# radian628/raymarching-engine

Measured on AMD Instinct MI355X. Metric: Mpixels/sec at 3840x2160 Mandelbulb, higher is better.
Workload: dtype f32

## Files before the change

include/hip_raymarch.h:

```cpp
#ifndef HIP_RAYMARCH_H
#define HIP_RAYMARCH_H

#include <stddef.h>
#include <stdint.h>

#ifndef RM_API
#define RM_API __attribute__((visibility("default")))
#endif

#ifdef __cplusplus
extern "C" {
#endif

#define RM_ABI_VERSION 8

#define RM_MAX_BOUNCES 10
#define RM_MAX_LIGHTS 10
#define RM_MAX_PRIMS 256

enum {
  RM_OK = 0,
  RM_ERR_INVALID = 1,
  RM_ERR_DEVICE = 2,
  RM_ERR_NO_DEVICE = 3
// ... 85 lines not shown
typedef struct RmSceneDesc {
  int32_t kind;
  int32_t nprims;
  const RmPrim* prims;
  float params[16];
  RmMaterial material;
  int32_t nsurfaces;
  int32_t reserved;
  const RmSurface* surfaces;
} RmSceneDesc;

RM_API void rm_material_default(RmMaterial* m);


typedef struct rm_ctx rm_ctx;
typedef struct rm_scene rm_scene;
typedef struct rm_fb rm_fb;

typedef struct RmRect {
  int32_t x, y, w, h;
} RmRect;

enum {
  RM_RENDER_STRICT = 0,
  RM_RENDER_FAST = 1,
  RM_RENDER_COLOR_ONLY = 2,
  RM_RENDER_MEGAKERNEL = 4,
  RM_RENDER_WAVEFRONT = 16,
  RM_RENDER_NO_COST_CLASSES = 8,
  RM_RENDER_NO_OVERLAP = 32,
  RM_RENDER_NO_FAR_JUMP = 64,
  RM_RENDER_NO_CULL = 128
};

enum { RM_PLANE_COLOR = 0, RM_PLANE_NORMAL_DOF = 1, RM_PLANE_ALBEDO_DEPTH = 2 };


RM_API int rm_ctx_create(int device, rm_ctx** out);
RM_API void rm_ctx_destroy(rm_ctx* ctx);
RM_API const char* rm_last_error(const rm_ctx* ctx);
RM_API int rm_ctx_set_stream(rm_ctx* ctx, void* hip_stream);
RM_API int rm_ctx_set_samples_in_flight(rm_ctx* ctx, int n);
RM_API const char* rm_ctx_last_warning(const rm_ctx* ctx);
RM_API int rm_ctx_set_sample_batch(rm_ctx* ctx, int n);
RM_API int rm_ctx_set_cost_order(rm_ctx* ctx, int on);
RM_API int rm_ctx_set_retire_eps(rm_ctx* ctx, float eps);
RM_API int rm_ctx_set_gl_stack(rm_ctx* ctx, int on);
RM_API int rm_ctx_set_cull_min_pixels(rm_ctx* ctx, long long pixels);
RM_API int rm_ctx_set_cull_budget(rm_ctx* ctx, size_t bytes);
RM_API int rm_ctx_cull_stats(const rm_ctx* ctx, unsigned long long* out4);
RM_API int rm_debug_counters(rm_ctx* ctx, unsigned long long* out16, int reset);

RM_API int rm_debug_cull_cell(const RmSceneDesc* desc, const double* centre, double radius, double margin, unsigned long long* out_words);
enum { RM_PIPELINE_NONE = 0, RM_PIPELINE_PIXEL_KERNEL = 1, RM_PIPELINE_WAVEFRONT = 2 };
RM_API int rm_ctx_last_pipeline(const rm_ctx* ctx);
RM_API int rm_device_memory(rm_ctx* ctx, size_t* free_bytes, size_t* total_bytes);
RM_API int rm_sync(rm_ctx* ctx);
RM_API int rm_abi_version(void);


RM_API int rm_scene_create(rm_ctx* ctx, const RmSceneDesc* desc, rm_scene** out);
RM_API void rm_scene_destroy(rm_scene* scene);


RM_API int rm_fb_create(rm_ctx* ctx, int width, int height, int row_begin, int row_count, rm_fb** out);
RM_API int rm_fb_create_striped(rm_ctx* ctx, int width, int height, int stripe_rows, int parts, int part,
                         void* color, void* normal_dof, void* albedo_depth, rm_fb** out);
RM_API int rm_fb_rows(const rm_fb* fb);
RM_API int rm_fb_width(const rm_fb* fb);
RM_API int rm_fb_height(const rm_fb* fb);
RM_API int rm_fb_wrap(rm_ctx* ctx, int width, int height, int row_begin, int row_count,
               void* color, void* normal_dof, void* albedo_depth, rm_fb** out);
RM_API int rm_fb_clear(rm_fb* fb);
RM_API void rm_fb_destroy(rm_fb* fb);
RM_API int rm_fb_download(rm_fb* fb, int plane, float* host);
RM_API int rm_fb_upload(rm_fb* fb, int plane, const float* host);
RM_API void* rm_fb_device_ptr(rm_fb* fb, int plane);

RM_API int rm_buffer_create(rm_ctx* ctx, size_t bytes, void** device_ptr);
RM_API int rm_buffer_destroy(rm_ctx* ctx, void* device_ptr);
RM_API int rm_buffer_download(rm_ctx* ctx, const void* device_ptr, void* host, size_t bytes);
RM_API int rm_buffer_upload(rm_ctx* ctx, void* device_ptr, const void* host, size_t bytes);


RM_API int rm_render_sample(rm_ctx* ctx, rm_scene* scene, rm_fb* fb, const RmUniforms* uniforms,
                     const RmRect* tile, int flags);

RM_API int rm_render_samples(rm_ctx* ctx, rm_scene* scene, rm_fb* fb, const RmUniforms* uniforms,
                      const float* rand_noise_pairs, int count, const RmRect* tile, int flags);

RM_API int rm_render_timed(rm_ctx* ctx, rm_scene* scene, rm_fb* fb, const RmUniforms* uniforms,
                    int count, const RmRect* tile, int flags, float* ms_per_launch);


enum { RM_PROBE_SDF = 0, RM_PROBE_CAST_RAY = 1, RM_PROBE_NORMAL = 2, RM_PROBE_MATERIAL = 3, RM_PROBE_CAST_STEPS = 4, RM_PROBE_CAST_SHADOW = 5 };
RM_API int rm_probe(rm_ctx* ctx, rm_scene* scene, int what, const float* in, int n, float param,
             int flags, float* out);

RM_API int rm_probe_camera(rm_ctx* ctx, const RmUniforms* uniforms, int width, int height, float* out);

RM_API int rm_probe_rng(rm_ctx* ctx, const RmUniforms* uniforms, int width, int height, int count, float* out);

enum { RM_MATH_SIN = 0, RM_MATH_COS = 1, RM_MATH_LOG = 2, RM_MATH_EXP = 3, RM_MATH_POW = 4, RM_MATH_ACOS = 5, RM_MATH_ATAN2 = 6, RM_MATH_TAN = 7,
       RM_MATH_POW_PAIR_NM1 = 8, RM_MATH_POW_PAIR_N = 9, RM_MATH_SINCOS_S = 10, RM_MATH_SINCOS_C = 11, RM_MATH_SQRT = 12, RM_MATH_DIV = 13, RM_MATH_COUNT = 14 };
RM_API int rm_probe_math(rm_ctx* ctx, int fn, const float* a, const float* b, int n, float* out);

// ... 25 lines not shown
```

raymarching-engine_amd/csrc/rm_api.hip:

```cpp
#include <hip/hip_runtime.h>

#include <cmath>
#include <cstdio>
#include <cstdlib>
#include <cstring>
#include <limits>
#include <mutex>
#include <new>
#include <string>
#include <unordered_map>
#include <vector>

#include "../../include/hip_raymarch.h"
#include "rm_params.hpp"

#ifndef RM_WITH_WAVEFRONT
#define RM_WITH_WAVEFRONT 0
#endif

#define RM_SP_MAX 8

extern "C" {
hipError_t rm_gl_launch_pixels(const void* kparams, hipStream_t stream);
hipError_t rm_gl_launch_probe(const void* probe_params, hipStream_t stream);
// ... 415 lines not shown
    reach = std::fmax(reach, std::fmax(std::fabs(lo[a]), std::fabs(hi[a])));
    build->centre[a] = 0.5 * (lo[a] + hi[a]);
  }
  half = 1.1 * half + kmax + 1e-3;
  if (!(half < 1e6) || !(reach < 1e6)) return false;
  int levels = 1;
  while (levels < RM_CULL_MAX_LEVELS && 1.2e-7 * (n + 8) * 1.74 * std::ldexp(half, levels) < 2.0 * half) levels++;
  if (smooth_spheres && levels > RM_CULL_SMOOTH_LEVELS) levels = RM_CULL_SMOOTH_LEVELS;
  build->half0 = half;
  build->reach = reach;
  build->nprims = n;
  const int cells = smooth_spheres ? (n >= 32 ? RM_CULL_N_SMOOTH : RM_CULL_N_SMOOTH / 2) : RM_CULL_N;
  build->n = cells;
  build->n_outer = smooth_spheres ? cells / RM_CULL_OUTER_DIV : cells;
  build->levels = levels;
  build->words = (n + 63) / 64;
  for (int a = 0; a < 3; a++) g->centre[a] = (float)build->centre[a];
  g->inv_half0 = (float)(1.0 / half);
  g->scale0 = (float)(cells / (2.0 * half));
  g->n = cells;
  g->n_outer = build->n_outer;
  g->levels = levels;
  g->words = build->words;
  return true;
}

int rm_debug_cull_cell(const RmSceneDesc* desc, const double* centre, double radius, double margin, unsigned long long* out_words) {
  if (!desc || !centre || !out_words || desc->kind != RM_SCENE_TABLE || desc->nprims < 1 || desc->nprims > RM_MAX_PRIMS || !desc->prims) return RM_ERR_INVALID;
  for (int i = 0; i < desc->nprims; i++) {
    const int type = desc->prims[i].type & 0xff;
    if ((type != RM_PRIM_SPHERE && type != RM_PRIM_BOX) || ((desc->prims[i].type >> 8) & 0xff) > RM_OP_INTERSECT) return RM_ERR_INVALID;
  }
  rm_cull_cell(desc->prims, desc->nprims, (desc->nprims + 63) / 64, centre, radius, margin, out_words);
  return RM_OK;
}

static void kifs_far_field(const RmSceneDesc* desc, DevScene* dev) {
  dev->far_end = 0;
  dev->far_r2 = 0.0f;
  const double iters = desc->params[RM_P_KIFS_ITERATIONS], s = desc->params[RM_P_KIFS_SCALE], off = std::fabs((double)desc->params[RM_P_KIFS_OFFSET]);
  if (!(s > 0.05 && s <= 0.9) || !(iters >= 0.0 && iters <= 64.0) || !(off < 1e6)) return;
  if (desc->kind == RM_SCENE_KIFS_BOX) {
    if (std::pow(s, std::ceil(iters)) < 1e-15) return;
    const double r = 2.0 * std::sqrt(3.0) * (off * s / (1.0 - s) + 1.0) + 1.0;
    dev->far_r2 = (float)(r * r);
    dev->far_end = 1;
  } else {
    const double r = 9999.0 + 1.01 * (off * s / (1.0 - s) + 1.0) + 2.0;
    dev->far_r2 = (float)(r * r);
    dev->far_end = 3;
  }
}

int rm_scene_create(rm_ctx* ctx, const RmSceneDesc* desc, rm_scene** out) {
  if (!ctx || !desc || !out) return fail(ctx, RM_ERR_INVALID, "rm_scene_create: NULL argument");
  *out = nullptr;
  char buf[256];
  if (desc->kind < 0 || desc->kind >= RM_SCENE_KIND_COUNT) {
    std::snprintf(buf, sizeof buf, "scene: unknown kind %d", desc->kind);
    return fail(ctx, RM_ERR_INVALID, buf);
  }
  if (!finite_all(desc->params, 16)) return fail(ctx, RM_ERR_INVALID, "scene: non-finite parameter");
  if (desc->material.sky_axis < 0 || desc->material.sky_axis > 2) return fail(ctx, RM_ERR_INVALID, "scene: material.sky_axis must be 0, 1 or 2");
  if (desc->nsurfaces < 0 || desc->nsurfaces > RM_MAX_SURFACES || (desc->nsurfaces > 0 && (!desc->surfaces || desc->kind != RM_SCENE_TABLE))) {
    std::snprintf(buf, sizeof buf, "scene: 0..%d surfaces, for a primitive table (got %d)", RM_MAX_SURFACES, desc->nsurfaces);
    return fail(ctx, RM_ERR_INVALID, buf);
  }
  for (int i = 0; i < desc->nsurfaces; i++)
    if (!finite_all(reinterpret_cast<const float*>(&desc->surfaces[i]), 12)) return fail(ctx, RM_ERR_INVALID, "scene: non-finite surface value");
  if (desc->kind == RM_SCENE_TABLE) {
    if (desc->nprims < 1 || desc->nprims > RM_MAX_PRIMS || !desc->prims) {
      std::snprintf(buf, sizeof buf, "scene: primitive table needs 1..%d rows (got %d)", RM_MAX_PRIMS, desc->nprims);
      return fail(ctx, RM_ERR_INVALID, buf);
    }
    int shapes = 0, kind_of_rows = -1;
    for (int i = 0; i < desc->nprims; i++) {
      const RmPrim& p = desc->prims[i];
      const int type = p.type & 0xff, op = (p.type >> 8) & 0xff;
      if (type > RM_PRIM_PLANE || op > RM_OP_SMOOTH_INTERSECT || (p.type >> 24) != 0) {
        std::snprintf(buf, sizeof buf, "scene: row %d: unknown primitive/operator 0x%x", i, p.type);
        return fail(ctx, RM_ERR_INVALID, buf);
      }
      const int surface = (p.type >> 16) & 0xff;
      if (type == RM_PRIM_KIND) {
        const int kind = (int)p.size[0];
        if ((float)kind != p.size[0] || (kind != RM_SCENE_MANDELBULB && kind != RM_SCENE_SPHERE_LATTICE)) {
          std::snprintf(buf, sizeof buf, "scene: row %d: a kind row evaluates RM_SCENE_MANDELBULB or RM_SCENE_SPHERE_LATTICE (size[0] = %g)", i, (double)p.size[0]);
          return fail(ctx, RM_ERR_INVALID, buf);
        }
        if (kind_of_rows >= 0 && kind_of_rows != kind) return fail(ctx, RM_ERR_INVALID, "scene: the kind rows of a table evaluate ONE kind (its parameters are the scene's parameter block)");
        kind_of_rows = kind;
        if (kind == RM_SCENE_MANDELBULB && !(desc->params[RM_P_BULB_ITERATIONS] >= 0.0f && desc->params[RM_P_BULB_ITERATIONS] <= 64.0f))
          return fail(ctx, RM_ERR_INVALID, "scene: mandelbulb iterations must be in 0..64");
        if (kind == RM_SCENE_SPHERE_LATTICE && !(desc->params[RM_P_LATTICE_PERIOD] > 0.0f)) return fail(ctx, RM_ERR_INVALID, "scene: the lattice's period must be > 0");
      }
      const bool shape = type != RM_PRIM_REPEAT && type != RM_PRIM_FOLD;
      if (surface > desc->nsurfaces || (surface != 0 && !shape)) {
        std::snprintf(buf, sizeof buf, "scene: row %d: surface %d of %d (only shape rows name a surface)", i, surface, desc->nsurfaces);
        return fail(ctx, RM_ERR_INVALID, buf);
      }
      if (!finite_all(p.center, 3) || !finite_all(p.size, 3) || !std::isfinite(p.k)) {
        std::snprintf(buf, sizeof buf, "scene: row %d: non-finite value", i);
        return fail(ctx, RM_ERR_INVALID, buf);
      }
      if (type == RM_PRIM_REPEAT && !(p.size[0] > 0.0f && p.size[1] > 0.0f && p.size[2] > 0.0f)) {
        std::snprintf(buf, sizeof buf, "scene: row %d: repeat needs a period > 0 on every axis", i);
// ... 2 lines not shown
      if (type == RM_PRIM_FOLD && !(p.k > 0.0f)) {
        std::snprintf(buf, sizeof buf, "scene: row %d: fold needs scale > 0", i);
        return fail(ctx, RM_ERR_INVALID, buf);
      }
      if (shape && (op == RM_OP_SMOOTH_UNION || op == RM_OP_SMOOTH_SUBTRACT || op == RM_OP_SMOOTH_INTERSECT) && !(p.k > 0.0f) && shapes > 0) {
        std::snprintf(buf, sizeof buf, "scene: row %d: smooth %s needs k > 0", i, op == RM_OP_SMOOTH_UNION ? "union" : op == RM_OP_SMOOTH_SUBTRACT ? "subtraction" : "intersection");
        return fail(ctx, RM_ERR_INVALID, buf);
      }
      if ((type == RM_PRIM_TORUS || type == RM_PRIM_CYLINDER) && !(p.size[0] >= 0.0f && p.size[1] >= 0.0f)) {
        std::snprintf(buf, sizeof buf, "scene: row %d: a torus / cylinder needs radii (and a half height) >= 0", i);
        return fail(ctx, RM_ERR_INVALID, buf);
      }
      if (type == RM_PRIM_PLANE && !(p.size[0] != 0.0f || p.size[1] != 0.0f || p.size[2] != 0.0f)) {
        std::snprintf(buf, sizeof buf, "scene: row %d: a plane needs a normal", i);
        return fail(ctx, RM_ERR_INVALID, buf);
      }
      shapes += shape ? 1 : 0;
    }
    if (shapes == 0) return fail(ctx, RM_ERR_INVALID, "scene: the table has no shape row (sphere / box), only domain operators");
  } else if (desc->kind == RM_SCENE_MANDELBULB) {
    if (!(desc->params[RM_P_BULB_ITERATIONS] >= 0.0f && desc->params[RM_P_BULB_ITERATIONS] <= 64.0f))
      return fail(ctx, RM_ERR_INVALID, "scene: mandelbulb iterations must be in 0..64");
  } else if (desc->kind == RM_SCENE_SPHERE_GRID || desc->kind == RM_SCENE_MENGER || desc->kind == RM_SCENE_KIFS_TREE ||
             desc->kind == RM_SCENE_KIFS_BOX) {
    const int slot = desc->kind == RM_SCENE_SPHERE_GRID ? RM_P_GRID_ITERATIONS : desc->kind == RM_SCENE_MENGER ? RM_P_MENGER_ITERATIONS : RM_P_KIFS_ITERATIONS;
    if (!(desc->params[slot] <= 64.0f)) return fail(ctx, RM_ERR_INVALID, "scene: fractal iterations must be <= 64");
  }
  rm_scene* s = new (std::nothrow) rm_scene();
  if (!s) return fail(ctx, RM_ERR_DEVICE, "out of host memory");
  s->ctx = ctx;
  s->dev.kind = desc->kind;
  s->dev.nprims = desc->kind == RM_SCENE_TABLE ? desc->nprims : 0;
  if (desc->kind == RM_SCENE_TABLE) {
    bool spheres_smooth = true, domain = false, boxes = false, surfaces = false, kinds = false, more = false;
    for (int i = 0; i < desc->nprims; i++) {
      const int type = desc->prims[i].type & 0xff, op = (desc->prims[i].type >> 8) & 0xff;
      if (((desc->prims[i].type >> 16) & 0xff) != 0) surfaces = true;
      if (type != RM_PRIM_SPHERE || (i > 0 && op != RM_OP_SMOOTH_UNION)) spheres_smooth = false;
      if (type == RM_PRIM_REPEAT || type == RM_PRIM_FOLD) domain = true;
      if (type == RM_PRIM_BOX || type == RM_PRIM_TORUS || type == RM_PRIM_CYLINDER || type == RM_PRIM_PLANE) boxes = true;
      if (type == RM_PRIM_KIND) kinds = true;
      if (type > RM_PRIM_KIND || op > RM_OP_INTERSECT) more = true;
    }
    s->dev.table_flags = (spheres_smooth ? RM_TABLE_SPHERES_SMOOTH : 0) | (domain ? RM_TABLE_HAS_DOMAIN : 0) | (boxes || kinds ? 0 : RM_TABLE_NO_BOXES) |
                         (surfaces ? RM_TABLE_HAS_SURFACES : 0) | (kinds ? RM_TABLE_HAS_KIND : 0) | (more ? RM_TABLE_MORE : 0);
    if (spheres_smooth && desc->nprims >= 2 && desc->nprims * 3 <= RM_MAX_PRIMS * 2) {
      bool one_k = true;
      for (int i = 2; i < desc->nprims; i++) one_k = one_k && desc->prims[i].k == desc->prims[1].k;
      if (one_k) s->dev.table_flags |= RM_TABLE_UNIFORM_K;
    }
  }
  if (desc->kind == RM_SCENE_TABLE) table_far_field(desc, &s->dev);
  if (desc->kind == RM_SCENE_KIFS_BOX || desc->kind == RM_SCENE_KIFS_TREE) kifs_far_field(desc, &s->dev);
  if (desc->kind == RM_SCENE_SPHERE_GRID) {
    const float* c = &desc->params[RM_P_GRID_CENTER];
    const double r = 2.0 * (std::sqrt((double)c[0] * c[0] + (double)c[1] * c[1] + (double)c[2] * c[2]) + std::fabs((double)desc->params[RM_P_GRID_BIG_SIZE])) + 1.0;
    if (r < 1e9) { s->dev.far_r2 = (float)(r * r); s->dev.far_end = 1; }
  }
  std::memcpy(s->dev.p, desc->params, sizeof s->dev.p);
  if (s->dev.table_flags & RM_TABLE_UNIFORM_K) {
    s->dev.p[0] = desc->prims[1].k;
    s->dev.p[1] = 0.5f * (1.0f / desc->prims[1].k);
  }
  s->dev.mat = desc->material;
  (void)hipSetDevice(ctx->device);
  if (s->dev.nprims > 0) {
    const size_t bytes = sizeof(RmPrim) * (size_t)s->dev.nprims;
    hipError_t e = hipMalloc(reinterpret_cast<void**>(&s->d_prims), bytes);
    if (e == hipSuccess) e = hipMemcpy(s->d_prims, desc->prims, bytes, hipMemcpyHostToDevice);
    if (e != hipSuccess) {
      if (s->d_prims) (void)hipFree(s->d_prims);
      delete s;
      return fail(ctx, RM_ERR_DEVICE, std::string("rm_scene_create: ") + hipGetErrorString(e));
    }
    s->dev.prims = s->d_prims;
  }
  if (desc->kind == RM_SCENE_TABLE) {
    CullGrid g;
    CullBuild build;
    if (table_cull_params(desc, &g, &build)) {
      s->cull_wanted = true;
      s->cull_grid = g;
      s->cull_build = build;
    }
  }
  if (s->dev.table_flags & RM_TABLE_HAS_SURFACES) {
    RmSurface all[RM_MAX_SURFACES + 1];
    const RmMaterial& m = desc->material;
    all[0] = RmSurface{{m.diffuse[0], m.diffuse[1], m.diffuse[2]}, m.roughness, {m.specular[0], m.specular[1], m.specular[2]}, m.subsurface,
                       {m.subsurface_color[0], m.subsurface_color[1], m.subsurface_color[2]}, m.ior};
    for (int i = 0; i < desc->nsurfaces; i++) all[i + 1] = desc->surfaces[i];
    const size_t bytes = sizeof(RmSurface) * (size_t)(desc->nsurfaces + 1);
    hipError_t e = hipMalloc(reinterpret_cast<void**>(&s->d_surfaces), bytes);
    if (e == hipSuccess) e = hipMemcpy(s->d_surfaces, all, bytes, hipMemcpyHostToDevice);
    if (e != hipSuccess) {
      if (s->d_surfaces) (void)hipFree(s->d_surfaces);
      if (s->d_prims) (void)hipFree(s->d_prims);
      delete s;
      return fail(ctx, RM_ERR_DEVICE, std::string("rm_scene_create: ") + hipGetErrorString(e));
    }
    s->dev.surfaces = s->d_surfaces;
    s->dev.nsurfaces = desc->nsurfaces;
  }
  *out = s;
  return RM_OK;
}
// ... 1088 lines not shown
```

raymarching-engine_amd/csrc/rm_device.hpp:

```cpp
#pragma once

#include <hip/hip_runtime.h>

#include "../../include/hip_raymarch.h"
#include "rm_params.hpp"

namespace rm {
#ifdef RM_LANE_STATS
static __device__ unsigned long long g_lane_stats[4];
#endif


#define RM_DEV __device__ __forceinline__

struct v3 {
  float x, y, z;
};

RM_DEV v3 V(float x, float y, float z) { return v3{x, y, z}; }
RM_DEV v3 operator+(v3 a, v3 b) { return V(a.x + b.x, a.y + b.y, a.z + b.z); }
RM_DEV v3 operator-(v3 a, v3 b) { return V(a.x - b.x, a.y - b.y, a.z - b.z); }
RM_DEV v3 operator*(v3 a, v3 b) { return V(a.x * b.x, a.y * b.y, a.z * b.z); }
RM_DEV v3 operator*(v3 a, float s) { return V(a.x * s, a.y * s, a.z * s); }
RM_DEV v3 adds(v3 a, float s) { return V(a.x + s, a.y + s, a.z + s); }
// ... 883 lines not shown
        else pow8_round_next(z, dr, pos, rho2, r2);
#ifdef RM_LANE_STATS
        rounds++;
#endif
      }
    } else {
      for (int i = 1; i < iterations; i++) {
        if (r2 > bail2) break;
        if (i == iterations - 1) dr = pow8_round_dr(dr, r2);
        else pow8_round_next(z, dr, pos, rho2, r2);
      }
    }
#ifdef RM_LANE_STATS
    lane_stats(rounds);
#endif
    return pow8_distance(r2, dr);
  }
#ifdef RM_LANE_STATS
  static RM_DEV void lane_stats(int rounds) {
    const unsigned long long act = ballot(true);
    unsigned long long lane_rounds = 0, wave_rounds = 0;
    for (int r = 1; r <= 8; r++) {
      const unsigned long long m = ballot(rounds >= r);
      lane_rounds += __popcll(m);
      wave_rounds += m != 0ull ? 1 : 0;
    }
    if ((int)__lane_id() == __ffsll((long long)act) - 1) {
      atomicAdd(&g_lane_stats[0], lane_rounds);
      atomicAdd(&g_lane_stats[1], wave_rounds * 64ull);
      atomicAdd(&g_lane_stats[2], (unsigned long long)__popcll(act));
      atomicAdd(&g_lane_stats[3], 64ull);
    }
  }
#endif
  static RM_DEV float eval_pow8(const DevScene& sc, v3 pos) {
    return (int)sc.p[RM_P_BULB_ITERATIONS] == 8 ? eval_pow8_n<8>(sc, pos) : eval_pow8_n<0>(sc, pos);
  }
  template <class M>
  static RM_DEV float eval(const DevScene& sc, const SceneLds&, v3 p) {
    if (M::fast && sc.p[RM_P_BULB_POWER] == 8.0f) return eval_pow8(sc, p);
    return eval_generic<M>(sc, p);
  }
  static constexpr int far_jump_steps = 30;
  static RM_DEV bool far_jump_applies(const DevScene& sc) { return sc.p[RM_P_BULB_ITERATIONS] >= 1.0f && sc.p[RM_P_BULB_BAILOUT] >= 0.0f; }
  static RM_DEV bool far_jump(const DevScene& sc, v3 p, v3 dir, int left, v3& end) {
    const float bail2 = sc.p[RM_P_BULB_BAILOUT] * sc.p[RM_P_BULB_BAILOUT];
    const float r2 = FM::fma(p.z, p.z, pow8_rho2(p));
    return far_jump_at(p, dir, left, r2, RM_BUILD_FAST && sc.p[RM_P_BULB_POWER] == 8.0f ? bail2 : 1.001f * bail2, end);
  }
  static RM_DEV bool far_jump_at(v3 p, v3 dir, int left, float r2, float bail2, v3& end) {
    if (!(r2 > gmax(bail2, 4.0f) && r2 < 1e30f) || left < (r2 >= 1e12f ? 16 : (r2 >= 1e4f ? 22 : far_jump_steps))) return false;
    const float s = dot<FM>(p, dir), dd = dot<FM>(dir, dir);
    if (!(s >= 0.0f && dd > 0.98f && dd < 1.02f)) return false;
    v3 e = dir * __builtin_inff();
    if (e.x != e.x || e.y != e.y || e.z != e.z) e = V(e.x + e.y + e.z, e.x + e.y + e.z, e.x + e.y + e.z);
    end = e;
    return true;
  }
  template <int ITERS>
  static RM_DEV bool pow8_eval_or_jump(const DevScene& sc, v3 p, v3 dir, int left, bool jump, float& d, v3& end) {
    const float bail2 = sc.p[RM_P_BULB_BAILOUT] * sc.p[RM_P_BULB_BAILOUT];
    const float rho2 = pow8_rho2(p);
    const float r2 = FM::fma(p.z, p.z, rho2);
    if (ITERS != 8 && (int)sc.p[RM_P_BULB_ITERATIONS] < 1) { d = pow8_distance(0.0f, 1.0f); return false; }
    if (r2 > bail2) {
      if (jump && far_jump_at(p, dir, left, r2, bail2, end)) return true;
#ifdef RM_LANE_STATS
      lane_stats(0);
#endif
      d = pow8_distance_far(r2);
      return false;
    }
    d = pow8_near<ITERS>(sc, p, rho2, r2, bail2);
    return false;
  }

  static constexpr bool has_cost_classes = true;
  static RM_DEV bool nonfinite_normal_is_nan(const DevScene&) { return true; }
  static constexpr int cheap_cap = 2;
  template <class M>
  static RM_DEV bool eval_cheap(const DevScene& sc, const SceneLds& lds, v3 p, float& d) {
    const int iterations = (int)sc.p[RM_P_BULB_ITERATIONS];
    if (iterations <= cheap_cap) { d = eval<M>(sc, lds, p); return true; }
    bool bailed = false;
    if (M::fast && sc.p[RM_P_BULB_POWER] == 8.0f) {
      const float bail2 = sc.p[RM_P_BULB_BAILOUT] * sc.p[RM_P_BULB_BAILOUT];
      v3 z = p;
      float dr = 1.0f, r2 = 0.0f;
      int rounds = 0;
      for (int i = 0; i <= cheap_cap; i++) {
        const float rho2 = pow8_rho2(z);
        r2 = FM::fma(z.z, z.z, rho2);
        if (r2 > bail2) { bailed = true; break; }
        if (i == cheap_cap) break;
        pow8_round(z, dr, p, rho2, r2);
        rounds++;
      }
      if (!bailed) return false;
      d = rounds == 0 ? pow8_distance_far(r2) : pow8_distance(r2, dr);
      return true;
    }
    const float power = sc.p[RM_P_BULB_POWER], bailout = sc.p[RM_P_BULB_BAILOUT];
    v3 z = p;
    float dr = 1.0f, r = 0.0f;
    for (int i = 0; i <= cheap_cap; i++) {
      r = M::sqrt_of_ordinary(dot<M>(z, z));
      if (r > bailout) { bailed = true; break; }
      if (i == cheap_cap) break;
      generic_round<M>(z, dr, p, r, power);
// ... 245 lines not shown
```

raymarching-engine_amd/csrc/rm_kernels.inc:

```

namespace rm {

template <int KIND, class M>
RM_DEV float march_sdf(const DevScene& sc, const SceneLds& lds, v3 p) {
#ifndef RM_FARFIELD_PM
#define RM_FARFIELD_PM 0
#endif
  if (M::fast && RM_FARFIELD_PM) {
    const bool far = !(gmax(fabsf(p.x), gmax(fabsf(p.y), fabsf(p.z))) <= 65536.0f);
    if (far) return Sdf<KIND>::template eval<PM>(sc, lds, p);
  }
  return Sdf<KIND>::template eval<M>(sc, lds, p);
}

template <int KIND, class M>
RM_DEV v3 cast_ray(const DevScene& sc, const SceneLds& lds, v3 p, v3 dir, float steps, float retire_eps, bool jump = true, int need_e = 1000) {
  bool done = false;
  if constexpr (!(ExactExits<M>::value && FarJump<KIND>::value)) jump = false;
  else jump = jump && Sdf<KIND>::far_jump_applies(sc);
  if constexpr (ExactExits<M>::value && IsBigTable<KIND>::value) {
    const int left0 = (int)gmin(ceilf(steps), 1048576.0f);
    const bool ask = jump && steps > 0.0f && Sdf<RM_SCENE_TABLE>::clear_miss_applies(sc, p, dir, left0);
    if (ballot(ask) != 0ull && ask && Sdf<RM_SCENE_TABLE>::clear_miss(sc, lds, p, dir, left0)) return Sdf<RM_SCENE_TABLE>::far_end_state(sc, dir);
  }
// ... 41 lines not shown

template <int KIND>
RM_DEV Surface surface_at(const DevScene& sc, const SceneLds& lds, v3 p) {
  if constexpr (IsTable<KIND>::value && KIND != RM_KIND_TABLE_SMOOTH) {
    if (sc.table_flags & RM_TABLE_HAS_SURFACES) {
      const int k = Sdf<KIND>::template surface_index<NM>(sc, lds, p);
      const float4 a = lds.surf[3 * k], b = lds.surf[3 * k + 1], c = lds.surf[3 * k + 2];
      return Surface{V(a.x, a.y, a.z), V(b.x, b.y, b.z), V(c.x, c.y, c.z), a.w, b.w, c.w};
    }
  }
  return scene_surface(sc);
}
template <int KIND>
RM_DEV bool has_surfaces(const DevScene& sc) { return IsTable<KIND>::value && KIND != RM_KIND_TABLE_SMOOTH && (sc.table_flags & RM_TABLE_HAS_SURFACES) != 0; }

#ifndef RM_REPACK_STEPS
#define RM_REPACK_STEPS 16
#endif
#ifndef RM_REPACK_STEPS_TABLE
#define RM_REPACK_STEPS_TABLE 8
#endif
template <int KIND> struct RepackSteps { static constexpr int value = IsTable<KIND>::value ? RM_REPACK_STEPS_TABLE : RM_REPACK_STEPS; };
#ifndef RM_REPACK_KIND_MASK
#define RM_REPACK_KIND_MASK ((1u << RM_SCENE_MANDELBULB) | (1u << RM_KIND_BULB8) | (1u << RM_SCENE_MENGER) | (1u << RM_KIND_TABLE_BIG) | (1u << RM_KIND_TABLE_SMOOTH))
#endif
template <int KIND>
struct BlockRepack {
  static constexpr bool value = ((RM_REPACK_KIND_MASK >> KIND) & 1u) != 0u;
};

#ifndef RM_REPACK_WAVES
#define RM_REPACK_WAVES(KIND) ((KIND) == RM_SCENE_MANDELBULB || (KIND) == RM_KIND_BULB8 || (KIND) == RM_KIND_TABLE_BIG || (KIND) == RM_KIND_TABLE_SMOOTH ? 8 : 4)
#endif
template <int KIND>
struct BlockShape {
  static constexpr int waves = BlockRepack<KIND>::value ? RM_REPACK_WAVES(KIND) : 4;
  static constexpr int wx = waves == 16 ? 4 : 2, wy = waves / wx;
  static constexpr bool can_lie = waves == 8;
  static constexpr int threads = waves * 64, px = wx * 8, py = wy * 8;
};

template <int WAVES>
struct MarchSharedT {
  static constexpr int N = WAVES > 0 ? WAVES * 64 : 1;
  float4 pos_i[N];
  float4 dir_steps[N];
  float4 result[N];
  int wave_count[WAVES > 0 ? WAVES : 1];
};


template <int KIND, class M>
RM_DEV v3 cast_ray_block(const DevScene& sc, const SceneLds& lds, MarchSharedT<0>&, v3 p0, v3 dir0, float steps0, float retire_eps,
                         bool, bool jump, int need_e = 1000) {
  return cast_ray<KIND, M>(sc, lds, p0, dir0, steps0, retire_eps, jump, need_e);
}

template <int KIND, class M, int WAVES>
RM_DEV v3 cast_ray_block(const DevScene& sc, const SceneLds& lds, MarchSharedT<WAVES>& sm, v3 p0, v3 dir0, float steps0, float retire_eps,
                         bool wanted, bool jump, int need_e = 1000) {
  if constexpr (!(ExactExits<M>::value && FarJump<KIND>::value)) jump = false;
  else jump = jump && Sdf<KIND>::far_jump_applies(sc);
  const int tid = threadIdx.x, wave = tid >> 6, lane = tid & 63;
  v3 p = p0, dir = dir0;
  int left = wanted && steps0 > 0.0f ? (int)ceilf(gmin(steps0, 16777216.0f)) : 0;
  int owner = tid;
  sm.result[tid] = make_float4(p0.x, p0.y, p0.z, 0.0f);
  if constexpr (ExactExits<M>::value && IsBigTable<KIND>::value) {
    const bool ask = jump && left > 0 && Sdf<RM_SCENE_TABLE>::clear_miss_applies(sc, p, dir, left);
    if (ballot(ask) != 0ull) {
      if (ask && Sdf<RM_SCENE_TABLE>::clear_miss(sc, lds, p, dir, left)) {
        const v3 e = Sdf<RM_SCENE_TABLE>::far_end_state(sc, dir);
        sm.result[tid] = make_float4(e.x, e.y, e.z, 0.0f);
        left = 0;
      }
    }
  }
  __syncthreads();
  auto step = [&](const v3& a, v3& b) {
    if constexpr (M::fast && FusedJump<KIND>::value && !RM_FARFIELD_PM) {
      if (left > 0) {
        float d;
        if (Sdf<KIND>::template eval_or_jump<M>(sc, lds, a, dir, left, jump, d, b)) {
          left = 0;
          sm.result[owner] = make_float4(b.x, b.y, b.z, 0.0f);
        } else {
          b = a + dir * d;
          bool done = same_bits(a, b);
          if (retire_eps > 0.0f) done = done || fabsf(d) <= retire_eps * gmax(1.0f, gmax(fabsf(b.x), gmax(fabsf(b.y), fabsf(b.z))));
          left = done ? 0 : left - 1;
          if (left <= 0) sm.result[owner] = make_float4(b.x, b.y, b.z, 0.0f);
        }
      }
      return;
    }
    if constexpr (ExactExits<M>::value && FarJump<KIND>::value) {
      if (jump && left > 0 && Sdf<KIND>::far_jump(sc, a, dir, left, b)) {
        left = 0;
        sm.result[owner] = make_float4(b.x, b.y, b.z, 0.0f);
      }
      if constexpr (IsBigTable<KIND>::value) {
        if (jump && left > 0 && need_e < 1000 && far_shadow_escape(a, dir, left, sc.far_r2, need_e, b)) {
          left = 0;
          sm.result[owner] = make_float4(b.x, b.y, b.z, 0.0f);
        }
      }
    }
    if (left > 0) {
      const float d = march_sdf<KIND, M>(sc, lds, a);
      b = a + dir * d;
      bool done = same_bits(a, b);
      if (M::fast && retire_eps > 0.0f)
        done = done || fabsf(d) <= retire_eps * gmax(1.0f, gmax(fabsf(b.x), gmax(fabsf(b.y), fabsf(b.z))));
      left = done ? 0 : left - 1;
      if (left <= 0) sm.result[owner] = make_float4(b.x, b.y, b.z, 0.0f);
    }
  };
  static_assert(RepackSteps<KIND>::value % 2 == 0, "the march body takes its steps in pairs");
#ifndef RM_REPACK_FIRST
#define RM_REPACK_FIRST 0
#endif
#ifndef RM_REPACK_RAMP
#define RM_REPACK_RAMP 0
#endif
  bool skip_march = RM_REPACK_FIRST != 0;
  int round_steps = RM_REPACK_RAMP > 0 ? RM_REPACK_RAMP : RepackSteps<KIND>::value;
  for (;;) {
    if (!skip_march && ballot(left > 0) != 0ull) {
// ... 269 lines not shown
      bool done = !(0.0f < steps);
      while (ballot(!done) != 0ull) {
        if (!done) done = preview_step<KIND, MM>(sc, lds, u, steps, retire_eps, ray);
      }
    }
    pos = ray.p;
    const float steps_taken = ray.steps_taken, depth = ray.depth;
    const float4 prev_color = P.color[pix];
    const float shade = 1.0f - steps_taken / steps;
    const Surface psf = surface_at<KIND>(sc, lds, pos);
    const v3 out = (cut_color(psf.diffuse, sc.mat.diffuse_cutoff, pos) + cut_color(psf.specular, sc.mat.specular_cutoff, pos)) * shade + scene_emission(sc, pos);
    float4 col;
    if (u.blendMode == 0) {
      const float f = u.blendWithPreviousFactor;
      col = make_float4(gmix<PM>(out.x, prev_color.x, f), gmix<PM>(out.y, prev_color.y, f), gmix<PM>(out.z, prev_color.z, f),
                        gmix<PM>(1.0f, prev_color.w, f));
    } else {
      col = make_float4(prev_color.x + out.x * u.exposure, prev_color.y + out.y * u.exposure,
                        prev_color.z + out.z * u.exposure, prev_color.w + 0.0f * u.exposure);
    }
    if (u.showDofFocalPlane != 0) {
      const float focus = fabsf(depth - u.dofFocalPlaneDistance) / depth;
      if (focus < u.dofFocalPlaneDistance * 0.005f) col = make_float4(1.0f, gmod<PM>(col.y + 0.5f, 1.0f), gmod<PM>(col.z + 0.5f, 1.0f), 1.0f);
    }
    if (valid) P.color[pix] = col;
    report_cost();
    return;
  }

#if RM_KARG_FRESH
#define RM_SCENE_HERE(name) const DevScene name = karg_load(&karg()->scene)
#define RM_KARGS(name) KArg* const name = karg()
#else
#define RM_SCENE_HERE(name) const DevScene& name = P.scene
#define RM_KARGS(name) const KParams* const name = &P
#endif
  v3 albedo = V(1.0f, 1.0f, 1.0f), light = V(0.0f, 0.0f, 0.0f);
  for (float i = 0.0f;; i += 1.0f) {
    RM_KARGS(K0);
    if (!(i < K0->u.reflections)) break;
    const v3 old = pos;
#ifndef RM_CULL_ALL_BOUNCES
#define RM_CULL_ALL_BOUNCES 0
#endif
    if constexpr (KIND == RM_KIND_TABLE_SMOOTH && !RM_CULL_ALL_BOUNCES) {
      if (i == 1.0f) {
        __syncthreads();
        if (threadIdx.x == 0) lds.cull_here = 0u;
        __syncthreads();
      }
    }
    {
      RM_SCENE_HERE(scm);
      pos = cast_ray_block<KIND, MM>(scm, lds, march_shared, pos, dir, K0->u.raymarchingStepCountsArray[(int)i], retire_eps, valid, K0->no_far_jump == 0);
    }
    RM_DIAG_EXIT(2, pos.x, pos.y, pos.z)
    RM_SCENE_HERE(sc);
    RM_KARGS(K);
    const float path_length = inv_exp_dist(uniform_sample(rng), K->u.fogDensity);
    light = light + albedo * scene_emission(sc, pos);
    v3 normal = scene_normal<KIND>(sc, lds, pos, 0.00001f);

    const bool escaped = distance<PM>(old, pos) > path_length || any_nonfinite(pos);
    const Surface sf = (!escaped && has_surfaces<KIND>(sc)) ? surface_at<KIND>(sc, lds, pos) : scene_surface(sc);
    v3 subsurf_pos = pos;
    if (!escaped) {
      const float subsurf = -1.0f / sf.subsurface * PM::log(1.0f - uniform_sample(rng));
      v3 sdir = normalize<PM>(sphere_sample(rng));
      sdir = normalize<PM>(V(gmix<PM>(dir.x, sdir.x, 1.0f), gmix<PM>(dir.y, sdir.y, 1.0f), gmix<PM>(dir.z, sdir.z, 1.0f)));
      sdir = sdir * -gsign(dot<PM>(sdir, normal));
      subsurf_pos = pos + sdir * subsurf;
    } else {
      rng_skip_uniform(rng);
      rng_skip_sphere(rng);
    }

    const v3 prev_albedo = albedo;
    v3 diffuse_col = cut_color(sf.diffuse, sc.mat.diffuse_cutoff, pos);
    v3 specular_col = cut_color(sf.specular, sc.mat.specular_cutoff, pos);
    v3 prev_dir = dir;

    if (escaped) {
      pos = old + dir * gmin(path_length, 1000000.0f);
      dir = sphere_sample(rng);
      diffuse_col = V(1.0f, 1.0f, 1.0f);
      specular_col = V(1.0f, 1.0f, 1.0f);
      prev_dir = dir;
    } else if (Sdf<KIND>::template eval<NM>(sc, lds, subsurf_pos) > 0.001f) {
      albedo = albedo * sf.subsurface_color;
      pos = subsurf_pos;
      const v3 sp = sphere_sample(rng);
      dir = normalize<PM>(V(gmix<PM>(dir.x, sp.x, 1.0f), gmix<PM>(dir.y, sp.y, 1.0f), gmix<PM>(dir.z, sp.z, 1.0f)));
    } else {
      const float db = length<PM>(diffuse_col), sb = length<PM>(specular_col);
      const float prob = (db > sb) ? (1.0f - sb / db / 2.0f) : (db / sb / 2.0f);
      if (uniform_sample(rng) < prob) {
        albedo = albedo * diffuse_col;
        const v3 nd = sphere_sample(rng);
        dir = nd * gsign(dot<PM>(normal, nd));
      } else {
        const float f = gclamp(schlick(-dot<PM>(dir, normal), 1.0f, sf.ior), 0.0f, 1.0f);
        albedo = albedo * (specular_col * f);
        const v3 rv = sphere_sample(rng);
        dir = reflect<PM>(dir, normal);
        const v3 axis = normalize<PM>(cross(rv, dir));
        dir = rodrigues(dir, axis, sf.roughness * uniform_sample(rng));
      }
// ... 471 lines not shown
```

raymarching-engine_amd/csrc/rm_params.hpp:

```cpp
#pragma once

#include <hip/hip_runtime.h>

#include "../../include/hip_raymarch.h"

#define RM_TABLE_SPHERES_SMOOTH 1
#define RM_TABLE_HAS_DOMAIN 2
#define RM_TABLE_NO_BOXES 8
#define RM_TABLE_UNIFORM_K 4
#define RM_TABLE_HAS_KIND 32
#define RM_TABLE_MORE 64
#define RM_TABLE_HAS_SURFACES 16

#define RM_BATCH_MAX 8

struct CullGrid {
  const unsigned long long* cells;
  float centre[3];
  float inv_half0;
  float scale0;
  int n, n_outer, levels, words;
};
struct CullBuild {
  const RmPrim* prims;
// ... 81 lines not shown
      const double k = 0.0;
      keep = !(lo_i >= U + margin);
      if (keep && best >= 0) {
        const CullRow& q = prims[best];
        const double sx = p.c[0] - q.c[0], sy = p.c[1] - q.c[1], sz = p.c[2] - q.c[2];
        const bool ps = p.shape == RM_PRIM_SPHERE, qs = q.shape == RM_PRIM_SPHERE;
        const double pe = p.reach, qe = q.reach;
        const double s = sqrt(sx * sx + sy * sy + sz * sz) + pe + qe;
        const double a = (ps ? di + p.size[0] : di) - rad, b = (qs ? best_d + q.size[0] : best_d) - rad;
        if (a > 0.0 && b > 0.0) {
          const double lip = fmin(2.0, s / sqrt(a * b));
          keep = !(di - best_d - rad * lip >= k + margin);
        }
      }
      U = fmin(U, hi_i);
      L = fmin(L, lo_i);
      if (best < 0 || di < best_d) { best = i; best_d = di; }
      if (keep) B = NONE;
    } else if (op == RM_OP_SUBTRACT) {
      keep = !(-lo_i <= L - margin);
      U = fmax(U, -lo_i);
      L = fmax(L, -hi_i);
      if (keep) best = -1, B = NONE;
    } else {
      keep = !(hi_i <= L - margin);
      U = fmax(U, hi_i);
      L = fmax(L, lo_i);
      if (keep) best = -1, B = NONE;
    }
    if (keep) out[i >> 6] |= 1ull << (i & 63);
  }
}

__host__ __device__ inline void rm_cull_cell(const RmPrim* prims, int nprims, int words, const double* c, double rad, double margin, unsigned long long* out) {
  CullRow rows[RM_MAX_PRIMS];
  for (int i = 0; i < nprims; i++) rows[i] = rm_cull_row(prims[i]);
  rm_cull_cell_rows(rows, nprims, words, c, rad, margin, out);
}

struct DevScene {
  int kind;
  int nprims;
  int table_flags;
  int reserved;
  const RmPrim* prims;
  float p[16];
  RmMaterial mat;
  const RmSurface* surfaces;
  int nsurfaces;
  int far_end;
  float far_r2;
  float clear_k;
  float clear_rho;
  CullGrid cull;
};

struct KParams {
  RmUniforms u;
  DevScene scene;
  float4* color;
  float4* normal_dof;
  float4* albedo_depth;
  int W, H;
  int row_begin;
  int stripe_rows, parts, part;
  int tx, ty, tw, th;
  float retire_eps;
  float4* stage;
  long long stage_stride;
  int batch;
  int tile_wide;
  float batch_noise[RM_BATCH_MAX][2];
  const unsigned int* block_order;
  unsigned int* block_cost;
  int no_far_jump;
};

#define RM_TABLE_BIG_ROWS 16
__host__ __device__ inline bool rm_table_big(const KParams& P) {
  return P.scene.kind == RM_SCENE_TABLE && P.scene.nprims >= RM_TABLE_BIG_ROWS && P.u.renderMode == 0 && !(P.scene.table_flags & RM_TABLE_HAS_KIND);
}

__host__ __device__ inline int rm_global_row(const KParams& P, int local) {
  if (P.stripe_rows <= 0) return P.row_begin + local;
  return ((local / P.stripe_rows) * P.parts + P.part) * P.stripe_rows + local % P.stripe_rows;
}

struct ProbeParams {
  DevScene scene;
  const float* in;
  float* out;
  int n;
  int what;
  float param;
  float retire_eps;
  int no_far_jump;
};

namespace rm {
enum {
  WF_POS = 0,
  WF_DIR,
  WF_OLD,
  WF_ALB,
  WF_LIG,
  WF_NRM,
// ... 56 lines not shown
```

raymarching-engine_amd/native.py:

```python
from __future__ import annotations

import ctypes as C
from pathlib import Path
from typing import Optional

import numpy as np

from . import abi
from .scene import Scene

import os

os.environ.setdefault("HSA_ENABLE_IPC_MODE_LEGACY", "0")

LIB_PATH = Path(os.environ.get("RM_LIB") or Path(__file__).resolve().parent / "libhip_raymarch.so")

EXPORTS = [
    "rm_abi_version", "rm_material_default", "rm_ctx_create", "rm_ctx_destroy", "rm_last_error", "rm_ctx_set_stream",
    "rm_ctx_set_retire_eps", "rm_ctx_set_samples_in_flight", "rm_ctx_last_warning", "rm_ctx_set_cost_order", "rm_ctx_set_cull_min_pixels", "rm_ctx_set_cull_budget", "rm_ctx_cull_stats", "rm_debug_counters", "rm_device_memory", "rm_sync", "rm_scene_create", "rm_scene_destroy", "rm_fb_create", "rm_fb_create_striped", "rm_fb_rows", "rm_fb_width", "rm_fb_height", "rm_fb_wrap", "rm_fb_clear", "rm_fb_destroy",
    "rm_fb_download", "rm_fb_upload", "rm_fb_device_ptr", "rm_buffer_create", "rm_buffer_destroy", "rm_buffer_download", "rm_buffer_upload", "rm_render_sample", "rm_render_samples", "rm_ctx_set_sample_batch", "rm_ctx_set_gl_stack", "rm_render_timed",
    "rm_probe", "rm_probe_camera", "rm_probe_rng", "rm_probe_math", "rm_assemble_striped", "rm_assemble_striped_bytes", "rm_present", "rm_present_planes", "rm_present_device", "rm_present_rows", "rm_pack_present_rows", "rm_ctx_last_pipeline", "rm_present_sharded", "rm_present_sharded_start", "rm_present_sharded_finish", "rm_present_striped_rows", "rm_debug_cull_cell",
]


def cull_cell(scene, centre, radius: float, margin: float = 0.0):
    lib = load_library()
    desc = scene.desc()
    words = (desc.nprims + 63) // 64
    out = (C.c_ulonglong * words)()
    c = (C.c_double * 3)(*[float(v) for v in centre])
    rc = lib.rm_debug_cull_cell(C.byref(desc), c, float(radius), float(margin), out)
    if rc != abi.RM_OK:
        raise RmError(rc, "rm_debug_cull_cell: not a table of shapes only")
    return [bool((out[i >> 6] >> (i & 63)) & 1) for i in range(desc.nprims)]


class RmError(RuntimeError):
    def __init__(self, code: int, message: str):
        super().__init__(message)
        self.code = code


_lib = None
_libs: dict = {}
XCHECK_LIB_PATH = Path(__file__).resolve().parent.parent / "tests" / "_xcheck" / "libhip_raymarch_xcheck.so"


def _share_torch_hip_runtime():
    import importlib.util
    import sys

    if "torch" in sys.modules:
        return
    try:
        spec = importlib.util.find_spec("torch")
    except (ImportError, ValueError):
        spec = None
    if spec is None or not spec.submodule_search_locations:
        return
    libdir = Path(list(spec.submodule_search_locations)[0]) / "lib"
    for name in ("libhsa-runtime64.so", "libamdhip64.so"):
        p = libdir / name
        if p.exists():
            try:
                C.CDLL(str(p), mode=C.RTLD_GLOBAL)
            except OSError:
                return


def load_library(path=None):
    global _lib
    path = Path(path) if path is not None else LIB_PATH
    if str(path) in _libs:
        return _libs[str(path)]
    if not path.exists():
        raise RmError(abi.RM_ERR_DEVICE, f"{path} is missing: build it with `python raymarching-engine_amd/build.py` "
                                          "(hipcc --offload-arch=gfx950); there is no CPU fallback")
    _share_torch_hip_runtime()
    lib = C.CDLL(str(path))
    vp, fp, ip = C.c_void_p, C.POINTER(C.c_float), C.c_int
    sig = {
        "rm_abi_version": (ip, []),
        "rm_material_default": (None, [C.POINTER(abi.RmMaterial)]),
        "rm_ctx_create": (ip, [ip, C.POINTER(vp)]),
        "rm_ctx_destroy": (None, [vp]),
        "rm_last_error": (C.c_char_p, [vp]),
        "rm_ctx_set_stream": (ip, [vp, vp]),
        "rm_ctx_set_retire_eps": (ip, [vp, C.c_float]),
        "rm_ctx_set_samples_in_flight": (ip, [vp, C.c_int]),
        "rm_ctx_last_warning": (C.c_char_p, [vp]),
        "rm_ctx_set_sample_batch": (ip, [vp, C.c_int]),
        "rm_ctx_set_gl_stack": (ip, [vp, C.c_int]),
        "rm_device_memory": (ip, [vp, C.POINTER(C.c_size_t), C.POINTER(C.c_size_t)]),
        "rm_buffer_create": (ip, [vp, C.c_size_t, C.POINTER(C.c_void_p)]),
        "rm_buffer_destroy": (ip, [vp, vp]),
        "rm_buffer_download": (ip, [vp, vp, vp, C.c_size_t]),
        "rm_buffer_upload": (ip, [vp, vp, vp, C.c_size_t]),
        "rm_ctx_set_cost_order": (ip, [vp, C.c_int]),
        "rm_ctx_set_cull_min_pixels": (ip, [vp, C.c_longlong]),
        "rm_ctx_set_cull_budget": (ip, [vp, C.c_size_t]),
        "rm_ctx_cull_stats": (ip, [vp, C.POINTER(C.c_ulonglong)]),
        "rm_debug_counters": (ip, [vp, C.POINTER(C.c_ulonglong), ip]),
        "rm_debug_cull_cell": (ip, [C.POINTER(abi.RmSceneDesc), C.POINTER(C.c_double), C.c_double, C.c_double, C.POINTER(C.c_ulonglong)]),
        "rm_sync": (ip, [vp]),
        "rm_scene_create": (ip, [vp, C.POINTER(abi.RmSceneDesc), C.POINTER(vp)]),
        "rm_scene_destroy": (None, [vp]),
        "rm_fb_create": (ip, [vp, ip, ip, ip, ip, C.POINTER(vp)]),
        "rm_fb_wrap": (ip, [vp, ip, ip, ip, ip, vp, vp, vp, C.POINTER(vp)]),
        "rm_fb_create_striped": (ip, [vp, ip, ip, ip, ip, ip, vp, vp, vp, C.POINTER(vp)]),
        "rm_fb_rows": (ip, [vp]),
        "rm_fb_width": (ip, [vp]),
        "rm_fb_height": (ip, [vp]),
        "rm_fb_clear": (ip, [vp]),
        "rm_fb_destroy": (None, [vp]),
        "rm_fb_download": (ip, [vp, ip, fp]),
        "rm_fb_upload": (ip, [vp, ip, fp]),
        "rm_fb_device_ptr": (vp, [vp, ip]),
        "rm_render_sample": (ip, [vp, vp, vp, C.POINTER(abi.RmUniforms), C.POINTER(abi.RmRect), ip]),
        "rm_render_samples": (ip, [vp, vp, vp, C.POINTER(abi.RmUniforms), fp, ip, C.POINTER(abi.RmRect), ip]),
        "rm_render_timed": (ip, [vp, vp, vp, C.POINTER(abi.RmUniforms), ip, C.POINTER(abi.RmRect), ip, fp]),
        "rm_probe": (ip, [vp, vp, ip, fp, ip, C.c_float, ip, fp]),
        "rm_probe_camera": (ip, [vp, C.POINTER(abi.RmUniforms), ip, ip, fp]),
        "rm_probe_rng": (ip, [vp, C.POINTER(abi.RmUniforms), ip, ip, ip, fp]),
        "rm_probe_math": (ip, [vp, ip, fp, fp, ip, fp]),
        "rm_assemble_striped": (ip, [vp, vp, ip, ip, ip, ip, ip, vp, vp]),
        "rm_assemble_striped_bytes": (ip, [vp, vp, ip, ip, C.c_longlong, ip, ip, vp, vp]),
        "rm_present_device": (ip, [vp, vp, vp, ip, ip, ip, vp, vp]),
        "rm_present_rows": (ip, [vp, vp, ip, vp, vp]),
        "rm_pack_present_rows": (ip, [vp, vp, vp, vp]),
        "rm_ctx_last_pipeline": (ip, [vp]),
        "rm_present_sharded": (ip, [C.POINTER(vp), C.POINTER(vp), ip, ip, ip, C.POINTER(C.c_uint8), C.c_size_t]),
        "rm_present_sharded_start": (ip, [C.POINTER(vp), C.POINTER(vp), ip, ip, ip]),
        "rm_present_sharded_finish": (ip, [C.POINTER(vp), ip, C.POINTER(C.c_uint8), C.c_size_t]),
        "rm_present_striped_rows": (ip, [vp, vp, vp, ip, ip, ip, ip, ip, ip, vp, vp]),
        "rm_present": (ip, [vp, vp, ip, C.POINTER(C.c_uint8)]),
        "rm_present_planes": (ip, [vp, vp, vp, ip, ip, ip, C.POINTER(C.c_uint8)]),
    }
    for name, (res, args) in sig.items():
        if name.startswith("rm_debug_") and not hasattr(lib, name) and os.environ.get("RM_LIB"):
            continue
        fn = getattr(lib, name)
        fn.restype, fn.argtypes = res, args
    _libs[str(path)] = lib
    if path == LIB_PATH:
        _lib = lib
    return lib


def present_sharded(contexts, framebuffers, samples: int, dof: bool) -> np.ndarray:
    n = len(contexts)
    assert n == len(framebuffers) and n >= 1
    cs = (C.c_void_p * n)(*[c.h for c in contexts])
    fs = (C.c_void_p * n)(*[f.h for f in framebuffers])
    out = np.empty((framebuffers[0].height, framebuffers[0].width, 4), np.uint8)
    contexts[0]._check(contexts[0].lib.rm_present_sharded(cs, fs, n, int(samples), 1 if dof else 0, out.ctypes.data_as(C.POINTER(C.c_uint8)), out.nbytes))
    return out
# ... 275 lines not shown
```

Baseline: 4536.

## Certify Mandelbulb ray escape analytically to skip marching for rays leaving the bulb

Computes, at scene creation, a conservative escape radius and step budget for the power-8 Mandelbulb using interval bounds on the distance estimator. In the fast pixel kernel, rays whose origin lies outside this certified radius and that point outward (or miss the sphere) are retired immediately to the far endpoint instead of being marched. The aim is to cut wasted steps for secondary or bounce rays that provably escape. It adds a per-ray check and relies on the bound being conservative for float rounding.

```diff
diff --git a/include/hip_raymarch.h b/include/hip_raymarch.h
--- a/include/hip_raymarch.h
+++ b/include/hip_raymarch.h
@@ -161,6 +161,7 @@
 RM_API int rm_debug_counters(rm_ctx* ctx, unsigned long long* out16, int reset);
 
 RM_API int rm_debug_cull_cell(const RmSceneDesc* desc, const double* centre, double radius, double margin, unsigned long long* out_words);
+RM_API int rm_debug_bulb_escape(float power, float iterations, float bailout, double* out6);
 enum { RM_PIPELINE_NONE = 0, RM_PIPELINE_PIXEL_KERNEL = 1, RM_PIPELINE_WAVEFRONT = 2 };
 RM_API int rm_ctx_last_pipeline(const rm_ctx* ctx);
 RM_API int rm_device_memory(rm_ctx* ctx, size_t* free_bytes, size_t* total_bytes);
diff --git a/raymarching-engine_amd/csrc/rm_api.hip b/raymarching-engine_amd/csrc/rm_api.hip
--- a/raymarching-engine_amd/csrc/rm_api.hip
+++ b/raymarching-engine_amd/csrc/rm_api.hip
@@ -491,6 +491,54 @@
   }
 }
 
+static int bulb_escape_bounds(float power, float iterations, float bailout, double out[6]) {
+  for (int i = 0; i < 6; i++) out[i] = 0.0;
+  if (!(power == 8.0f && iterations >= 2.0f && bailout >= 2.0f && bailout <= 64.0f)) return 0;
+  const double B = bailout, rel = 1e-3;
+  double lo = 1.0, hi = B;
+  for (int i = 0; i < 200; i++) {
+    const double mid = 0.5 * (lo + hi);
+    ((std::pow(mid, 8.0) - mid) * (1.0 - rel) >= B * (1.0 + rel) ? hi : lo) = mid;
+  }
+  const double R = hi, Bp = B * (1.0 + rel);
+  double dmin = HUGE_VAL;
+  const int pieces = 4096;
+  for (int i = 0; i < pieces; i++) {
+    const double a = R + (Bp - R) * i / pieces, b = R + (Bp - R) * (i + 1) / pieces;
+    const double r1 = (std::pow(a, 8.0) - a) * (1.0 - rel);
+    dmin = std::fmin(dmin, 0.5 * std::log(r1) * r1 / (8.0 * std::pow(b, 7.0) + 1.0));
+  }
+  const double delta = 0.9 * dmin, delta_out = 0.9 * 0.5 * std::log(B) * B;
+  const double o_max = 4.0 * B, dir_min = std::sqrt(0.98);
+  const double n = std::ceil(o_max / (dir_min * delta_out)) + 1.0 + std::ceil(2.0 * Bp / (dir_min * delta)) + 1.0 + 2.0;
+  const double m = 0.01 + n * o_max * std::ldexp(1.0, -20);
+  const double steps = n + 30.0;
+  out[0] = R; out[1] = delta; out[2] = delta_out; out[3] = m; out[4] = o_max; out[5] = steps;
+  return 1;
+}
+
+static void bulb_escape_field(const RmSceneDesc* desc, DevScene* dev) {
+  double b[6];
+  dev->esc_b2 = 0.0f;
+  dev->esc_o2 = 0.0f;
+  dev->esc_steps = 0;
+  if (!bulb_escape_bounds(desc->params[RM_P_BULB_POWER], desc->params[RM_P_BULB_ITERATIONS], desc->params[RM_P_BULB_BAILOUT], b)) return;
+  const double e = (b[0] + b[3]) * (b[0] + b[3]);
+  float ef = (float)e;
+  if ((double)ef < e) ef = std::nextafter(ef, HUGE_VALF);
+  float of = (float)(b[4] * b[4]);
+  if ((double)of > b[4] * b[4]) of = std::nextafter(of, 0.0f);
+  dev->esc_b2 = ef;
+  dev->esc_o2 = of;
+  dev->esc_steps = (int)b[5];
+}
+
+int rm_debug_bulb_escape(float power, float iterations, float bailout, double* out6) {
+  if (!out6) return RM_ERR_INVALID;
+  bulb_escape_bounds(power, iterations, bailout, out6);
+  return RM_OK;
+}
+
 int rm_scene_create(rm_ctx* ctx, const RmSceneDesc* desc, rm_scene** out) {
   if (!ctx || !desc || !out) return fail(ctx, RM_ERR_INVALID, "rm_scene_create: NULL argument");
   *out = nullptr;
@@ -599,6 +647,7 @@
   }
   if (desc->kind == RM_SCENE_TABLE) table_far_field(desc, &s->dev);
   if (desc->kind == RM_SCENE_KIFS_BOX || desc->kind == RM_SCENE_KIFS_TREE) kifs_far_field(desc, &s->dev);
+  if (desc->kind == RM_SCENE_MANDELBULB) bulb_escape_field(desc, &s->dev);
   if (desc->kind == RM_SCENE_SPHERE_GRID) {
     const float* c = &desc->params[RM_P_GRID_CENTER];
     const double r = 2.0 * (std::sqrt((double)c[0] * c[0] + (double)c[1] * c[1] + (double)c[2] * c[2]) + std::fabs((double)desc->params[RM_P_GRID_BIG_SIZE])) + 1.0;
diff --git a/raymarching-engine_amd/csrc/rm_device.hpp b/raymarching-engine_amd/csrc/rm_device.hpp
--- a/raymarching-engine_amd/csrc/rm_device.hpp
+++ b/raymarching-engine_amd/csrc/rm_device.hpp
@@ -959,9 +959,19 @@
     if (!(r2 > gmax(bail2, 4.0f) && r2 < 1e30f) || left < (r2 >= 1e12f ? 16 : (r2 >= 1e4f ? 22 : far_jump_steps))) return false;
     const float s = dot<FM>(p, dir), dd = dot<FM>(dir, dir);
     if (!(s >= 0.0f && dd > 0.98f && dd < 1.02f)) return false;
+    end = far_end(dir);
+    return true;
+  }
+  static RM_DEV v3 far_end(v3 dir) {
     v3 e = dir * __builtin_inff();
     if (e.x != e.x || e.y != e.y || e.z != e.z) e = V(e.x + e.y + e.z, e.x + e.y + e.z, e.x + e.y + e.z);
-    end = e;
+    return e;
+  }
+  static RM_DEV bool escape_certified(const DevScene& sc, v3 o, v3 dir, int left, v3& end) {
+    const float o2 = dot<FM>(o, o), s = dot<FM>(o, dir), dd = dot<FM>(dir, dir), e = sc.esc_b2;
+    if (!(e > 0.0f && left >= sc.esc_steps && o2 >= e && o2 <= sc.esc_o2 && dd > 0.98f && dd < 1.02f)) return false;
+    if (!(s >= 0.0f || (o2 - e) * dd >= s * s)) return false;
+    end = far_end(dir);
     return true;
   }
   template <int ITERS>
diff --git a/raymarching-engine_amd/csrc/rm_kernels.inc b/raymarching-engine_amd/csrc/rm_kernels.inc
--- a/raymarching-engine_amd/csrc/rm_kernels.inc
+++ b/raymarching-engine_amd/csrc/rm_kernels.inc
@@ -117,13 +117,13 @@
 
 template <int KIND, class M>
 RM_DEV v3 cast_ray_block(const DevScene& sc, const SceneLds& lds, MarchSharedT<0>&, v3 p0, v3 dir0, float steps0, float retire_eps,
-                         bool, bool jump, int need_e = 1000) {
+                         bool, bool jump, int need_e = 1000, bool = false) {
   return cast_ray<KIND, M>(sc, lds, p0, dir0, steps0, retire_eps, jump, need_e);
 }
 
 template <int KIND, class M, int WAVES>
 RM_DEV v3 cast_ray_block(const DevScene& sc, const SceneLds& lds, MarchSharedT<WAVES>& sm, v3 p0, v3 dir0, float steps0, float retire_eps,
-                         bool wanted, bool jump, int need_e = 1000) {
+                         bool wanted, bool jump, int need_e = 1000, bool certify = false) {
   if constexpr (!(ExactExits<M>::value && FarJump<KIND>::value)) jump = false;
   else jump = jump && Sdf<KIND>::far_jump_applies(sc);
   const int tid = threadIdx.x, wave = tid >> 6, lane = tid & 63;
@@ -139,6 +139,13 @@
         sm.result[tid] = make_float4(e.x, e.y, e.z, 0.0f);
         left = 0;
       }
+    }
+  }
+  if constexpr (M::fast && FusedJump<KIND>::value && !RM_FARFIELD_PM) {
+    v3 e;
+    if (certify && jump && !(retire_eps > 0.0f) && left > 0 && Sdf<KIND>::escape_certified(sc, p, dir, left, e)) {
+      sm.result[tid] = make_float4(e.x, e.y, e.z, 0.0f);
+      left = 0;
     }
   }
   __syncthreads();
@@ -514,7 +521,8 @@
     }
     {
       RM_SCENE_HERE(scm);
-      pos = cast_ray_block<KIND, MM>(scm, lds, march_shared, pos, dir, K0->u.raymarchingStepCountsArray[(int)i], retire_eps, valid, K0->no_far_jump == 0);
+      pos = cast_ray_block<KIND, MM>(scm, lds, march_shared, pos, dir, K0->u.raymarchingStepCountsArray[(int)i], retire_eps, valid, K0->no_far_jump == 0,
+                                     1000, true);
     }
     RM_DIAG_EXIT(2, pos.x, pos.y, pos.z)
     RM_SCENE_HERE(sc);
diff --git a/raymarching-engine_amd/csrc/rm_params.hpp b/raymarching-engine_amd/csrc/rm_params.hpp
--- a/raymarching-engine_amd/csrc/rm_params.hpp
+++ b/raymarching-engine_amd/csrc/rm_params.hpp
@@ -157,6 +157,9 @@
   float far_r2;
   float clear_k;
   float clear_rho;
+  float esc_b2;
+  float esc_o2;
+  int esc_steps;
   CullGrid cull;
 };
 
diff --git a/raymarching-engine_amd/native.py b/raymarching-engine_amd/native.py
--- a/raymarching-engine_amd/native.py
+++ b/raymarching-engine_amd/native.py
@@ -20,6 +20,7 @@
     "rm_ctx_set_retire_eps", "rm_ctx_set_samples_in_flight", "rm_ctx_last_warning", "rm_ctx_set_cost_order", "rm_ctx_set_cull_min_pixels", "rm_ctx_set_cull_budget", "rm_ctx_cull_stats", "rm_debug_counters", "rm_device_memory", "rm_sync", "rm_scene_create", "rm_scene_destroy", "rm_fb_create", "rm_fb_create_striped", "rm_fb_rows", "rm_fb_width", "rm_fb_height", "rm_fb_wrap", "rm_fb_clear", "rm_fb_destroy",
     "rm_fb_download", "rm_fb_upload", "rm_fb_device_ptr", "rm_buffer_create", "rm_buffer_destroy", "rm_buffer_download", "rm_buffer_upload", "rm_render_sample", "rm_render_samples", "rm_ctx_set_sample_batch", "rm_ctx_set_gl_stack", "rm_render_timed",
     "rm_probe", "rm_probe_camera", "rm_probe_rng", "rm_probe_math", "rm_assemble_striped", "rm_assemble_striped_bytes", "rm_present", "rm_present_planes", "rm_present_device", "rm_present_rows", "rm_pack_present_rows", "rm_ctx_last_pipeline", "rm_present_sharded", "rm_present_sharded_start", "rm_present_sharded_finish", "rm_present_striped_rows", "rm_debug_cull_cell",
+    "rm_debug_bulb_escape",
 ]
 
 
@@ -33,6 +34,15 @@
     if rc != abi.RM_OK:
         raise RmError(rc, "rm_debug_cull_cell: not a table of shapes only")
     return [bool((out[i >> 6] >> (i & 63)) & 1) for i in range(desc.nprims)]
+
+
+def bulb_escape(power: float, iterations: float, bailout: float):
+    lib = load_library()
+    out = (C.c_double * 6)()
+    rc = lib.rm_debug_bulb_escape(float(power), float(iterations), float(bailout), out)
+    if rc != abi.RM_OK:
+        raise RmError(rc, "rm_debug_bulb_escape")
+    return dict(zip(("R", "delta", "delta_out", "margin", "o_max", "steps"), list(out)))
 
 
 class RmError(RuntimeError):
@@ -102,6 +112,7 @@
         "rm_ctx_cull_stats": (ip, [vp, C.POINTER(C.c_ulonglong)]),
         "rm_debug_counters": (ip, [vp, C.POINTER(C.c_ulonglong), ip]),
         "rm_debug_cull_cell": (ip, [C.POINTER(abi.RmSceneDesc), C.POINTER(C.c_double), C.c_double, C.c_double, C.POINTER(C.c_ulonglong)]),
+        "rm_debug_bulb_escape": (ip, [C.c_float, C.c_float, C.c_float, C.POINTER(C.c_double)]),
         "rm_sync": (ip, [vp]),
         "rm_scene_create": (ip, [vp, C.POINTER(abi.RmSceneDesc), C.POINTER(vp)]),
         "rm_scene_destroy": (None, [vp]),
```

Result: no change. 4560 (median of 6 runs) (+0.5%).
